# arneschneuing/DiffSBDD

Measured on NVIDIA H100. Metric: ligand_atoms_per_sec_500step_ddpm, higher is better.
Workload: dtype f32

## Files before the change

### diffsbdd_b200/csrc/dsb_tc.cu

```cuda
#include "dsb_tc.cuh"

namespace dsb {
using namespace tc;

__global__ void pack_b_image_kernel(float* __restrict__ hi, float* __restrict__ lo, const float* __restrict__ src, int lds,
                                    int scol, int n_rows, int n_dst_off, int K, int chunks, int TN) {
  const int64_t idx = (int64_t)blockIdx.x * blockDim.x + threadIdx.x;
  if (idx >= (int64_t)n_rows * K) return;
  const int n = (int)(idx / K), k = (int)(idx - (int64_t)n * K);
  const int nd = n_dst_off + n, nt = nd / TN, nl = nd % TN;
  const int kc = k / TKC, c = (k % TKC) >> 2, j = k & 3;
  const size_t off = ((size_t)nt * chunks + kc) * (size_t)(TN * TKC) + sw128_offset(nl, c) / 4 + j;
  const float w = src[(size_t)n * lds + scol + k];
  const float h = tf32_hi(w);
  hi[off] = h;
  lo[off] = w - h;
}

void launch_pack_b_image(float* hi, float* lo, const float* src, int lds, int scol, int n_rows, int n_dst_off, int K, int tn) {
  const int64_t tot = (int64_t)n_rows * K;
  pack_b_image_kernel<<<(unsigned)((tot + 255) / 256), 256>>>(hi, lo, src, lds, scol, n_rows, n_dst_off, K, K / TKC, tn);
}

__global__ void pack_b_image_f16_kernel(__half* __restrict__ hi, __half* __restrict__ lo, const float* __restrict__ src, int lds,
                                        int scol, int n_rows, int n_dst_off, int K, int chunks, float scale, int TN) {
  const int64_t idx = (int64_t)blockIdx.x * blockDim.x + threadIdx.x;
  if (idx >= (int64_t)n_rows * K) return;
  const int n = (int)(idx / K), k = (int)(idx - (int64_t)n * K);
  const int nd = n_dst_off + n, nt = nd / TN, nl = nd % TN;
  const int kc = k / TKC16, c16 = (k % TKC16) >> 3, j = k & 7;
  const size_t off = ((size_t)nt * chunks + kc) * (size_t)(TN * 64) + sw128_offset(nl, c16) / 2 + j;
  const float w = src[(size_t)n * lds + scol + k] * scale;
  const __half h = __float2half_rn(w);
  hi[off] = h;
  lo[off] = __float2half_rn(w - __half2float(h));
}

void launch_pack_b_image_f16(float* hi, float* lo, const float* src, int lds, int scol, int n_rows, int n_dst_off, int K, float scale, int tn) {
  const int64_t tot = (int64_t)n_rows * K;
  pack_b_image_f16_kernel<<<(unsigned)((tot + 255) / 256), 256>>>(reinterpret_cast<__half*>(hi), reinterpret_cast<__half*>(lo), src,
                                                                  lds, scol, n_rows, n_dst_off, K, K / TKC16, scale, tn);
}

__global__ void absmax_kernel(const float* __restrict__ src, int lds, int scol, int n_rows, int K, unsigned* __restrict__ out) {
  const int64_t idx = (int64_t)blockIdx.x * blockDim.x + threadIdx.x;
  float v = 0.f;
  if (idx < (int64_t)n_rows * K) { const int n = (int)(idx / K), k = (int)(idx - (int64_t)n * K); v = fabsf(src[(size_t)n * lds + scol + k]); }
#pragma unroll
  for (int o = 16; o > 0; o >>= 1) v = fmaxf(v, __shfl_xor_sync(0xffffffffu, v, o));
  if ((threadIdx.x & 31) == 0) atomicMax(out, __float_as_uint(v));
}
void launch_absmax(const float* src, int lds, int scol, int n_rows, int K, unsigned* out) {
  const int64_t tot = (int64_t)n_rows * K;
  absmax_kernel<<<(unsigned)((tot + 255) / 256), 256>>>(src, lds, scol, n_rows, K, out);
}

constexpr size_t kControlBytes = 128;
static_assert(sizeof(Control) <= kControlBytes, "Control block grew");
__device__ __forceinline__ char* align1024(uint8_t* raw) {
  return reinterpret_cast<char*>(raw) + ((1024u - (smem_u32(raw) & 1023u)) & 1023u);
}
template <int H> constexpr size_t tc_smem_base() { return 1024 + (size_t)NSTAGE * Geo<H>::STAGE_BYTES + kControlBytes; }

struct TcGemmArgs {
  const float* A1; int lda1; int K1;
  const float* A2; int lda2; int K2; float div2; const int32_t* deg2;
  const float* Bhi; const float* Blo;
  const float* bias; const float* R; int ldr;
  float* C; int ldc; int M; int Nn; int act;
  float* Z; int ldz;
  int dead_mt; int dead_nt;
  float inv_scale;
};

struct TileMap {
  int ntn, ntm, dead_mt, dead_nt, nA, n_live;
  __device__ TileMap(int M, int Nn, int dmt, int dnt, int TN) {
    ntn = Nn / TN; ntm = (M + TM - 1) / TM;
    dead_nt = dnt; dead_mt = dnt > 0 ? (dmt < ntm ? dmt : ntm) : ntm;
    nA = dead_mt * ntn;
    n_live = nA + (ntm - dead_mt) * (ntn - dead_nt);
  }
  __device__ void get(int t, int& mt, int& nt) const {
    if (t < nA) { mt = t / ntn; nt = t - mt * ntn; }
    else { const int u = t - nA, w = ntn - dead_nt; mt = dead_mt + u / w; nt = dead_nt + (u - (u / w) * w); }
  }
};

template <bool F16, int H>
__global__ void __launch_bounds__(TC_THREADS, 1) tc_node_gemm_kernel(TcGemmArgs g) {
  using G = Geo<H>;
  constexpr int TN = H, HPC = F16 ? 2 : 1;
  extern __shared__ uint8_t smem_raw[];
  char* const stages = align1024(smem_raw);
  Control* ctl = reinterpret_cast<Control*>(stages + NSTAGE * G::STAGE_BYTES);
  const int wg = threadIdx.x >> 7, warp = (threadIdx.x >> 5) & 3, lane = threadIdx.x & 31;
  const TileMap tm(g.M, g.Nn, g.dead_mt, g.dead_nt, TN);
  const int n_tiles = tm.n_live;
  const int n_my = ((int)blockIdx.x < n_tiles) ? (n_tiles - (int)blockIdx.x + (int)gridDim.x - 1) / (int)gridDim.x : 0;
  if (n_my == 0) return;
  const int K = g.K1 + g.K2, chunks = K / (F16 ? TKC16 : TKC);
  const uint32_t total = (uint32_t)(n_my * chunks);
  pdl_trigger();
  if (threadIdx.x == 0) control_init(ctl);
  __syncthreads();
  pdl_wait();
  const WeightStream<H> wst{ctl, stages};
  auto issue_w = [&](uint32_t q) {
    const int it = (int)(q / chunks), kc = (int)(q - (uint32_t)it * chunks);
    int mt, nt;
    tm.get(blockIdx.x + it * gridDim.x, mt, nt);
    const size_t off = ((size_t)nt * chunks + kc) * G::B_CHUNK_FLOATS;
    wst.issue(q, g.Bhi + off, g.Blo + off);
  };
  if (threadIdx.x >= MMA_THREADS) {
    regs_dec<WEIGHT_WG_REGS>();
    if (threadIdx.x == MMA_THREADS)
      for (uint32_t q = 0; q < total; ++q) issue_w(q);
    return;
  }
  regs_inc<MMA_WG_REGS>();

  const int sr = lane >> 3, pc = lane & 7;
  const int r0 = wg * WG_ROWS + 16 * warp + 4 * sr;
  const int re = wg * WG_ROWS + 16 * warp + (lane >> 2);
  const bool divides = g.div2 != 1.0f || g.deg2 != nullptr;
  float acc[G::ACC];
  MmaTracker trk;
  uint32_t q = 0;
  for (int it = 0; it < n_my; ++it) {
    int mt, nt;
    tm.get(blockIdx.x + it * gridDim.x, mt, nt);
    const int m0 = mt * TM, n0 = nt * TN;
    for (int kc = 0; kc < chunks; ++kc, ++q) {
      const int s = q & 1;
      char* st = stages + (size_t)s * G::STAGE_BYTES;
#pragma unroll
      for (int h = 0; h < HPC; ++h) {
        const int hf = kc * HPC + h, k = hf * TKC + 4 * pc;
        const bool second = k >= g.K1;
        float4 v[4];
#pragma unroll
        for (int i = 0; i < 4; ++i) {
          const int m = m0 + r0 + i;
          v[i] = make_float4(0.f, 0.f, 0.f, 0.f);
          if (m < g.M) v[i] = second ? *reinterpret_cast<const float4*>(g.A2 + (size_t)m * g.lda2 + (k - g.K1))
                                     : *reinterpret_cast<const float4*>(g.A1 + (size_t)m * g.lda1 + k);
        }
#pragma unroll
        for (int i = 0; i < 4; ++i) {
          float4 x = v[i];
          if (second && divides) {
            const int m = m0 + r0 + i;
            const float dv = g.deg2 ? (float)max(m < g.M ? g.deg2[m] : 1, 1) : g.div2;
            x.x = __fdiv_rn(x.x, dv); x.y = __fdiv_rn(x.y, dv); x.z = __fdiv_rn(x.z, dv); x.w = __fdiv_rn(x.w, dv);
          }
          store_pair<F16>(st + piece_offset<F16>(r0 + i, hf, pc), pk2(x.x, x.y), pk2(x.z, x.w));
        }
      }
      fence_proxy_async();
      wg_sync(wg);
      mbar_wait(&ctl->full_w[s], (q >> 1) & 1);
      wgmma_fence();
      mma_chunk<F16, H>(acc, st, wg, kc == 0);
      wgmma_commit();
      trk.after_commit<H>(ctl, acc, (int)q, kc == chunks - 1, lane == 0);
    }
    const f32x2 ip = pk2(g.inv_scale, g.inv_scale);
#pragma unroll
    for (int j = 0; j < H / 8; ++j) {
      const int n = n0 + 8 * j + 2 * (lane & 3);
      const f32x2 b = g.bias ? *reinterpret_cast<const float2*>(g.bias + n) : pk2(0.f, 0.f);
#pragma unroll
      for (int hh = 0; hh < 2; ++hh) {
        f32x2 x = pk2(acc[4 * j + 2 * hh], acc[4 * j + 2 * hh + 1]);
        x = F16 ? fma2(x, ip, b) : add2(x, b);
        if (g.act == 1) x = silu2(x);
        upk2(x, acc[4 * j + 2 * hh], acc[4 * j + 2 * hh + 1]);
      }
    }
    acc_fence(acc);
#pragma unroll
    for (int j = 0; j < H / 8; ++j) {
      const int n = n0 + 8 * j + 2 * (lane & 3);
#pragma unroll
      for (int hh = 0; hh < 2; ++hh) {
        const int row = m0 + re + 8 * hh;
        if (row < g.M) {
          f32x2 x = pk2(acc[4 * j + 2 * hh], acc[4 * j + 2 * hh + 1]);
          if (g.R) x = add2(*reinterpret_cast<const float2*>(g.R + (size_t)row * g.ldr + n), x);
          *reinterpret_cast<float2*>(g.C + (size_t)row * g.ldc + n) = x;
          if (g.Z) *reinterpret_cast<float2*>(g.Z + (size_t)row * g.ldz + n) = make_float2(0.f, 0.f);
        }
      }
    }
  }
}

template <int H>
struct EdgeExtra {
  float vec[2][3 * H];
  float wa[H];
  float d2[TM], d0[TM];
  int row[TM], col[TM], type[TM];
  float dir[3][TM];
};

struct TcEdgeArgs {
  const float* P; int ldp;
  const float4* x; const float4* cent; const int32_t* gid;
  const int32_t* vrow_ptr; const int32_t* vmap; int n_rows;
  const int32_t *erow, *ecol; const float* ed0; int NL;
  int nm;
  const float* W2hi[2]; const float* W2lo[2];
  const float* wr[2]; const float* wr0[2]; const float* tb[2]; const float* b2[2];
  const float* wa; const float* ba;
  float norm_constant, coords_range; int use_tanh;
  float* agg;
  float4* xagg;
  float inv_scale[2];
  float* part;
  int vcap;
};

template <bool COORD, int H>
__device__ __forceinline__ void edge_scalars(const TcEdgeArgs& a, EdgeExtra<H>* ex, int pr, int v0, int V, int m) {
  const int vr = v0 + pr;
  const int e = vr < V ? a.vmap[vr] : -1;
  int r = -1, c = 0, ty = 0; float d2 = 0.f, d0 = 0.f;
  float dir[3] = {0.f, 0.f, 0.f};
  if (e >= 0) {
    r = a.erow[e]; c = a.ecol[e]; d0 = a.ed0[e];
    const float4 xi = a.x[r], xj = a.x[c];
    const float dx = xi.x - xj.x, dy = xi.y - xj.y, dz = xi.z - xj.z;
    d2 = dx * dx + dy * dy + dz * dz;
    ty = (r < a.NL) == (c < a.NL) ? (r < a.NL ? 1 : 2) : 0;
    if (COORD) {
      if (m == 0) {
        const float den = sqrtf(d2 + 1e-8f) + a.norm_constant;
        dir[0] = dx / den; dir[1] = dy / den; dir[2] = dz / den;
      } else {
        const float4 mu = a.cent[a.gid[r]];
        const float ax = xi.x - mu.x, ay = xi.y - mu.y, az = xi.z - mu.z;
        const float bx = xj.x - mu.x, by = xj.y - mu.y, bz = xj.z - mu.z;
        const float cx = ay * bz - az * by, cy = az * bx - ax * bz, cz = ax * by - ay * bx;
        const float cn = sqrtf(cx * cx + cy * cy + cz * cz) + a.norm_constant;
        dir[0] = cx / cn; dir[1] = cy / cn; dir[2] = cz / cn;
      }
    }
  }
  ex->row[pr] = r; ex->col[pr] = c; ex->d2[pr] = d2; ex->d0[pr] = d0; ex->type[pr] = ty;
  if (COORD) {
#pragma unroll
    for (int k = 0; k < 3; ++k) ex->dir[k][pr] = dir[k];
  }
}

template <bool COORD, bool F16, int H, bool TB, bool DET = false>
__global__ void __launch_bounds__(TC_THREADS, 1) tc_edge_kernel(TcEdgeArgs a) {
  using G = Geo<H>;
  constexpr int HPC = F16 ? 2 : 1;
  constexpr int chunks = H / (TKC * HPC);
  extern __shared__ uint8_t smem_raw[];
  char* const stages = align1024(smem_raw);
  Control* ctl = reinterpret_cast<Control*>(stages + NSTAGE * G::STAGE_BYTES);
  EdgeExtra<H>* ex = reinterpret_cast<EdgeExtra<H>*>(reinterpret_cast<char*>(ctl) + kControlBytes);
  const int wg = threadIdx.x >> 7, wt = threadIdx.x & 127, warp = (threadIdx.x >> 5) & 3, lane = threadIdx.x & 31;
  const int nm = a.nm;

  pdl_trigger();
  for (int i = threadIdx.x; i < H; i += TC_THREADS) {
    for (int m = 0; m < nm; ++m) {
      float* v = ex->vec[m];
      v[i] = a.wr[m][i]; v[H + i] = a.wr0[m][i]; v[2 * H + i] = a.b2[m][i];
    }
    ex->wa[i] = a.wa ? a.wa[i] : 0.f;
  }
  if (threadIdx.x == 0) control_init(ctl);
  __syncthreads();
  pdl_wait();
  const int E = DET ? min(a.vrow_ptr[a.n_rows], a.vcap) : a.vrow_ptr[a.n_rows];
  const int n_units = ((E + TM - 1) / TM) * nm;
  const int n_my = ((int)blockIdx.x < n_units) ? (n_units - (int)blockIdx.x + (int)gridDim.x - 1) / (int)gridDim.x : 0;
  if (n_my == 0) return;
  auto unit_tile = [&](int j, int& m) { const int v = blockIdx.x + j * gridDim.x, t = v / nm; m = v - t * nm; return t; };
  const uint32_t total = (uint32_t)(n_my * chunks);
  const WeightStream<H> wst{ctl, stages};
  auto issue_w = [&](uint32_t q) {
    const int j = (int)(q / chunks), kc = (int)(q - (uint32_t)j * chunks);
    int m;
    unit_tile(j, m);
    wst.issue(q, a.W2hi[m] + (size_t)kc * G::B_CHUNK_FLOATS, a.W2lo[m] + (size_t)kc * G::B_CHUNK_FLOATS);
  };
  if (threadIdx.x >= MMA_THREADS) {
    regs_dec<WEIGHT_WG_REGS>();
    if (threadIdx.x == MMA_THREADS)
      for (uint32_t q = 0; q < total; ++q) issue_w(q);
    return;
  }
  regs_inc<MMA_WG_REGS>();

  const bool has_att = (!COORD) && a.wa != nullptr;
  const float ba = has_att ? a.ba[0] : 0.f;
  const int sr = lane >> 3, pc = lane & 7;
  const int r0 = wg * WG_ROWS + 16 * warp + 4 * sr;
  const int re = wg * WG_ROWS + 16 * warp + (lane >> 2);
  const float* const Pt = a.P + 4 * pc;
  const int soff = nm * H;
  float acc[G::ACC];
  MmaTracker trk;
  uint32_t q = 0;
  for (int j = 0; j < n_my; ++j) {
    int m;
    const int e0 = unit_tile(j, m) * TM;
    wg_sync(wg);
    if (wt < WG_ROWS) edge_scalars<COORD, H>(a, ex, wg * WG_ROWS + wt, e0, E, m);
    wg_sync(wg);
    const int moff = m * H;
    const float* pr = Pt + (size_t)max(ex->row[r0], 0) * a.ldp + moff;
    const float* ps[4];
    float pd2[4], pd0[4];
    int pty[4];
#pragma unroll
    for (int i = 0; i < 4; ++i) {
      ps[i] = Pt + (size_t)ex->col[r0 + i] * a.ldp + (soff + moff);
      pd2[i] = ex->d2[r0 + i]; pd0[i] = ex->d0[r0 + i];
      pty[i] = TB ? ex->type[r0 + i] * H : 0;
    }
    const float* wr = ex->vec[m] + 4 * pc;
    const float* wr0 = wr + H;
    const float* tbm = TB ? a.tb[m] + 4 * pc : nullptr;
#pragma unroll 1
    for (int kc = 0; kc < chunks; ++kc, ++q) {
      const int s = q & 1;
      char* st = stages + (size_t)s * G::STAGE_BYTES;
#pragma unroll
      for (int h = 0; h < HPC; ++h) {
        const int hf = kc * HPC + h;
        const float4 ga = *reinterpret_cast<const float4*>(pr + hf * TKC);
        float4 gb[4];
#pragma unroll
        for (int i = 0; i < 4; ++i) gb[i] = *reinterpret_cast<const float4*>(ps[i] + hf * TKC);
        const float4 r4 = *reinterpret_cast<const float4*>(wr + hf * TKC);
        const float4 r04 = *reinterpret_cast<const float4*>(wr0 + hf * TKC);
        const f32x2 a01 = pk2(ga.x, ga.y), a23 = pk2(ga.z, ga.w);
#pragma unroll
        for (int i = 0; i < 4; ++i) {
          const f32x2 d2p = pk2(pd2[i], pd2[i]), d0p = pk2(pd0[i], pd0[i]);
          f32x2 u01 = fma2(d0p, pk2(r04.x, r04.y), fma2(d2p, pk2(r4.x, r4.y), add2(a01, pk2(gb[i].x, gb[i].y))));
          f32x2 u23 = fma2(d0p, pk2(r04.z, r04.w), fma2(d2p, pk2(r4.z, r4.w), add2(a23, pk2(gb[i].z, gb[i].w))));
          if (TB) {
            const float4 t4 = *reinterpret_cast<const float4*>(tbm + pty[i] + hf * TKC);
            u01 = add2(u01, pk2(t4.x, t4.y)); u23 = add2(u23, pk2(t4.z, t4.w));
          }
          silu_pair<(DSB_SILU_PAIR & 1) != 0, (DSB_SILU_QUAD & 1) != 0>(u01, u23);
          store_pair<F16>(st + piece_offset<F16>(r0 + i, hf, pc), u01, u23);
        }
      }
      fence_proxy_async();
      wg_sync(wg);
      mbar_wait(&ctl->full_w[s], (q >> 1) & 1);
      wgmma_fence();
      mma_chunk<F16, H>(acc, st, wg, kc == 0);
      wgmma_commit();
      trk.after_commit<H>(ctl, acc, (int)q, kc == chunks - 1, lane == 0);
    }

    const float* b2 = ex->vec[m] + 2 * H;
    const f32x2 ip = pk2(a.inv_scale[m], a.inv_scale[m]);
    float s_lo = 0.f, s_hi = 0.f;
#pragma unroll
    for (int jj = 0; jj < H / 8; ++jj) {
      const int c = 8 * jj + 2 * (lane & 3);
      const f32x2 bb = *reinterpret_cast<const float2*>(b2 + c);
      const float2 ww = *reinterpret_cast<const float2*>(ex->wa + c);
      f32x2 lo = pk2(acc[4 * jj], acc[4 * jj + 1]), hi = pk2(acc[4 * jj + 2], acc[4 * jj + 3]);
      lo = F16 ? fma2(lo, ip, bb) : add2(lo, bb);
      hi = F16 ? fma2(hi, ip, bb) : add2(hi, bb);
      silu_pair<(DSB_SILU_PAIR & 2) != 0, (DSB_SILU_QUAD & 2) != 0>(lo, hi);
      upk2(lo, acc[4 * jj], acc[4 * jj + 1]); upk2(hi, acc[4 * jj + 2], acc[4 * jj + 3]);
      s_lo = fmaf(lo.y, ww.y, fmaf(lo.x, ww.x, s_lo));
      s_hi = fmaf(hi.y, ww.y, fmaf(hi.x, ww.x, s_hi));
    }
    s_lo += __shfl_xor_sync(0xffffffffu, s_lo, 1); s_lo += __shfl_xor_sync(0xffffffffu, s_lo, 2);
    s_hi += __shfl_xor_sync(0xffffffffu, s_hi, 1); s_hi += __shfl_xor_sync(0xffffffffu, s_hi, 2);
    const int row_lo = ex->row[re], row_hi = ex->row[re + 8];
    const int crow_lo = ex->row[re & ~3], crow_hi = ex->row[(re + 8) & ~3];
    const bool chunk_lane = (lane & 12) == 0;
    if constexpr (!COORD) {
      float g_lo = has_att ? sigmoid_f(s_lo + ba) : 1.0f, g_hi = has_att ? sigmoid_f(s_hi + ba) : 1.0f;
      g_lo = row_lo >= 0 ? g_lo : 0.f;
      g_hi = row_hi >= 0 ? g_hi : 0.f;
      float* const dst_lo = DET ? a.part + (size_t)((e0 + (re & ~3)) / kRowChunk) * H + 2 * (lane & 3)
                                : a.agg + (size_t)max(crow_lo, 0) * H + 2 * (lane & 3);
      float* const dst_hi = DET ? a.part + (size_t)((e0 + ((re + 8) & ~3)) / kRowChunk) * H + 2 * (lane & 3)
                                : a.agg + (size_t)max(crow_hi, 0) * H + 2 * (lane & 3);
#pragma unroll
      for (int jj = 0; jj < H / 8; ++jj) {
        float v0 = g_lo * acc[4 * jj], v1 = g_lo * acc[4 * jj + 1], v2 = g_hi * acc[4 * jj + 2], v3 = g_hi * acc[4 * jj + 3];
        v0 += __shfl_xor_sync(0xffffffffu, v0, 4); v1 += __shfl_xor_sync(0xffffffffu, v1, 4);
        v2 += __shfl_xor_sync(0xffffffffu, v2, 4); v3 += __shfl_xor_sync(0xffffffffu, v3, 4);
        v0 += __shfl_xor_sync(0xffffffffu, v0, 8); v1 += __shfl_xor_sync(0xffffffffu, v1, 8);
        v2 += __shfl_xor_sync(0xffffffffu, v2, 8); v3 += __shfl_xor_sync(0xffffffffu, v3, 8);
        if constexpr (DET)
          asm volatile("{\n\t.reg .pred p;\n\tsetp.ne.b32 p, %5, 0;\n\t"
                       "@p st.global.v2.f32 [%0], {%1, %2};\n\t"
                       "@p st.global.v2.f32 [%3], {%4, %6};\n\t}"
                       ::"l"(dst_lo + 8 * jj), "f"(v0), "f"(v1), "l"(dst_hi + 8 * jj), "f"(v2), "r"((int)chunk_lane), "f"(v3) : "memory");
        else
          asm volatile("{\n\t.reg .pred p;\n\tsetp.ne.b32 p, %5, 0;\n\t"
                       "@p red.global.add.v2.f32 [%0], {%1, %2};\n\t"
                       "@p red.global.add.v2.f32 [%3], {%4, %6};\n\t}"
                       ::"l"(dst_lo + 8 * jj), "f"(v0), "f"(v1), "l"(dst_hi + 8 * jj), "f"(v2), "r"((int)chunk_lane), "f"(v3) : "memory");
      }
    } else {
#pragma unroll
      for (int hh = 0; hh < 2; ++hh) {
        const int r = re + 8 * hh;
        const float sv = hh ? s_hi : s_lo;
        const bool live = (hh ? row_hi : row_lo) >= 0;
        float tr[3];
#pragma unroll
        for (int k = 0; k < 3; ++k) {
          const float d = ex->dir[k][r];
          float t;
          if (m == 0) t = a.use_tanh ? (d * tanhf(sv)) * a.coords_range : d * sv;
          else t = d * (a.use_tanh ? tanhf(sv) * a.coords_range : sv);
          t = live ? t : 0.f;
          t += __shfl_xor_sync(0xffffffffu, t, 4);
          t += __shfl_xor_sync(0xffffffffu, t, 8);
          tr[k] = t;
        }
        const int crow = hh ? crow_hi : crow_lo;
        if constexpr (DET) {
          if (chunk_lane && (lane & 3) == 0)
            reinterpret_cast<float4*>(a.part)[(size_t)((e0 + (r & ~3)) / kRowChunk) * nm + m] = make_float4(tr[0], tr[1], tr[2], 0.f);
        } else if (chunk_lane && (lane & 3) == 0 && crow >= 0) {
#pragma unroll
          for (int k = 0; k < 3; ++k) atomicAdd(reinterpret_cast<float*>(a.xagg) + (size_t)crow * 4 + k, tr[k]);
        }
      }
    }
  }
}

template <int H> static size_t gemm_smem_bytes() { return tc_smem_base<H>(); }
template <int H> static size_t edge_smem_bytes() {
  static_assert(tc_smem_base<H>() + sizeof(EdgeExtra<H>) <= 232448, "edge kernel exceeds the 227 KB of shared memory per CTA");
  return tc_smem_base<H>() + sizeof(EdgeExtra<H>);
}

bool tc_width_supported(int H) { return H == 128 || H == 192 || H == 256; }

template <typename Fn>
static int dispatch_width(int H, Fn&& fn) {
  switch (H) {
    case 128: return fn.template operator()<128>();
    case 192: return fn.template operator()<192>();
    case 256: return fn.template operator()<256>();
    default: set_error("tensor-core kernels exist for hidden_nf 128, 192, 256 (got %d)", H); return DSB_ERR_UNSUPPORTED_CONFIG;
  }
}

int configure_tc_kernels(int H) {
  return dispatch_width(H, [&]<int W>() -> int {
    const int gs = (int)gemm_smem_bytes<W>(), es = (int)edge_smem_bytes<W>();
    DSB_CUDA_OK(cudaFuncSetAttribute(tc_node_gemm_kernel<false, W>, cudaFuncAttributeMaxDynamicSharedMemorySize, gs));
    DSB_CUDA_OK(cudaFuncSetAttribute(tc_node_gemm_kernel<true, W>, cudaFuncAttributeMaxDynamicSharedMemorySize, gs));
    DSB_CUDA_OK(cudaFuncSetAttribute(tc_edge_kernel<false, false, W, false>, cudaFuncAttributeMaxDynamicSharedMemorySize, es));
    DSB_CUDA_OK(cudaFuncSetAttribute(tc_edge_kernel<false, false, W, true>, cudaFuncAttributeMaxDynamicSharedMemorySize, es));
    DSB_CUDA_OK(cudaFuncSetAttribute(tc_edge_kernel<false, true, W, false>, cudaFuncAttributeMaxDynamicSharedMemorySize, es));
    DSB_CUDA_OK(cudaFuncSetAttribute(tc_edge_kernel<false, true, W, true>, cudaFuncAttributeMaxDynamicSharedMemorySize, es));
    DSB_CUDA_OK(cudaFuncSetAttribute(tc_edge_kernel<true, false, W, false>, cudaFuncAttributeMaxDynamicSharedMemorySize, es));
    DSB_CUDA_OK(cudaFuncSetAttribute(tc_edge_kernel<true, false, W, true>, cudaFuncAttributeMaxDynamicSharedMemorySize, es));
    DSB_CUDA_OK(cudaFuncSetAttribute(tc_edge_kernel<true, true, W, false>, cudaFuncAttributeMaxDynamicSharedMemorySize, es));
    DSB_CUDA_OK(cudaFuncSetAttribute(tc_edge_kernel<true, true, W, true>, cudaFuncAttributeMaxDynamicSharedMemorySize, es));
    DSB_CUDA_OK(cudaFuncSetAttribute(tc_edge_kernel<false, false, W, false, true>, cudaFuncAttributeMaxDynamicSharedMemorySize, es));
    DSB_CUDA_OK(cudaFuncSetAttribute(tc_edge_kernel<false, false, W, true, true>, cudaFuncAttributeMaxDynamicSharedMemorySize, es));
    DSB_CUDA_OK(cudaFuncSetAttribute(tc_edge_kernel<false, true, W, false, true>, cudaFuncAttributeMaxDynamicSharedMemorySize, es));
    DSB_CUDA_OK(cudaFuncSetAttribute(tc_edge_kernel<false, true, W, true, true>, cudaFuncAttributeMaxDynamicSharedMemorySize, es));
    DSB_CUDA_OK(cudaFuncSetAttribute(tc_edge_kernel<true, false, W, false, true>, cudaFuncAttributeMaxDynamicSharedMemorySize, es));
    DSB_CUDA_OK(cudaFuncSetAttribute(tc_edge_kernel<true, false, W, true, true>, cudaFuncAttributeMaxDynamicSharedMemorySize, es));
    DSB_CUDA_OK(cudaFuncSetAttribute(tc_edge_kernel<true, true, W, false, true>, cudaFuncAttributeMaxDynamicSharedMemorySize, es));
    DSB_CUDA_OK(cudaFuncSetAttribute(tc_edge_kernel<true, true, W, true, true>, cudaFuncAttributeMaxDynamicSharedMemorySize, es));
    return 0;
  });
}

int launch_tc_node_gemm(const dsb_dynamics* d, const GemmArgs& g, const TcImage& w, int n_tile_off, bool f16, int32_t* status,
                        cudaStream_t s) {
  (void)status;
  if (g.M == 0) return 0;
  const int K = g.K1 + g.K2, TN = d->cfg.hidden_nf;
  if ((g.Nn % TN) || (K % TKC16) || (g.K1 % TKC16) || (g.lda1 % 4) || (g.ldc % 4)) {
    set_error("tc_node_gemm: unsupported shape K1=%d K2=%d Nn=%d", g.K1, g.K2, g.Nn);
    return DSB_ERR_INVALID_ARGUMENT;
  }
  TcGemmArgs a;
  a.A1 = g.A1; a.lda1 = g.lda1; a.K1 = g.K1; a.A2 = g.A2; a.lda2 = g.lda2; a.K2 = g.K2; a.div2 = g.div2; a.deg2 = g.deg2;
  const size_t img_off = (size_t)n_tile_off * (K / (f16 ? TKC16 : TKC)) * (size_t)(TN * TKC);
  a.Bhi = (f16 ? w.h_hi : w.t_hi) + img_off; a.Blo = (f16 ? w.h_lo : w.t_lo) + img_off;
  a.Z = g.Z; a.ldz = g.ldz;
  a.dead_nt = g.dead_cols / TN; a.dead_mt = a.dead_nt > 0 ? (g.dead_rows_from + TM - 1) / TM : 0;
  a.bias = g.bias; a.R = g.R; a.ldr = g.ldr; a.C = g.C; a.ldc = g.ldc; a.M = g.M; a.Nn = g.Nn; a.act = g.act;
  a.inv_scale = f16 ? w.h_inv : 1.0f;
  const int ntn_ = g.Nn / TN, ntm_ = (g.M + TM - 1) / TM;
  const int dmt_ = a.dead_nt > 0 ? (a.dead_mt < ntm_ ? a.dead_mt : ntm_) : ntm_;
  const int n_tiles = dmt_ * ntn_ + (ntm_ - dmt_) * (ntn_ - a.dead_nt);
  const int grid = n_tiles < d->num_sms ? n_tiles : d->num_sms;
  return dispatch_width(TN, [&]<int W>() -> int {
    DSB_CUDA_OK(launch_k(f16 ? tc_node_gemm_kernel<true, W> : tc_node_gemm_kernel<false, W>, grid, TC_THREADS, gemm_smem_bytes<W>(), s, a));
    return 0;
  });
}

int launch_tc_edge_gcl(const dsb_dynamics* d, const Dims& dm, const Workspace& ws, const GclW& w, const float4* x, PView pv, bool f16,
                       int32_t* status, cudaStream_t s) {
  (void)status;
  TcEdgeArgs a = {};
  a.P = pv.P; a.ldp = pv.ldp; a.x = x; a.cent = ws.cent; a.gid = ws.gid; a.vrow_ptr = ws.vrow_ptr; a.vmap = ws.vmap; a.n_rows = dm.N;
  a.erow = ws.erow; a.ecol = ws.ecol; a.ed0 = ws.ed0; a.NL = dm.NL; a.nm = 1;
  a.W2hi[0] = f16 ? w.iW2.h_hi : w.iW2.t_hi; a.W2lo[0] = f16 ? w.iW2.h_lo : w.iW2.t_lo;
  a.inv_scale[0] = f16 ? w.iW2.h_inv : 1.0f; a.inv_scale[1] = 1.0f;
  a.wr[0] = w.wr; a.wr0[0] = w.wr0; a.tb[0] = w.tb; a.b2[0] = w.b2;
  a.wa = w.wa; a.ba = w.ba; a.agg = ws.agg; a.part = ws.part; a.vcap = ws.vcap;
  const bool det = d->deterministic != 0;
  return dispatch_width(d->cfg.hidden_nf, [&]<int W>() -> int {
    auto kern = w.tb ? (f16 ? tc_edge_kernel<false, true, W, true> : tc_edge_kernel<false, false, W, true>)
                     : (f16 ? tc_edge_kernel<false, true, W, false> : tc_edge_kernel<false, false, W, false>);
    if (det)
      kern = w.tb ? (f16 ? tc_edge_kernel<false, true, W, true, true> : tc_edge_kernel<false, false, W, true, true>)
                  : (f16 ? tc_edge_kernel<false, true, W, false, true> : tc_edge_kernel<false, false, W, false, true>);
    DSB_CUDA_OK(launch_k(kern, d->num_sms, TC_THREADS, edge_smem_bytes<W>(), s, a));
    return 0;
  });
}

int launch_tc_edge_coord(const dsb_dynamics* d, const Dims& dm, const Workspace& ws, const EquivW& w, const float4* x, PView pv, bool f16,
                         int32_t* status, cudaStream_t s) {
  (void)status;
  const dsb_config& c = d->cfg;
  TcEdgeArgs a = {};
  a.nm = c.reflection_equivariant ? 1 : 2;
  a.P = pv.P; a.ldp = pv.ldp; a.x = x; a.cent = ws.cent; a.gid = ws.gid; a.vrow_ptr = ws.vrow_ptr; a.vmap = ws.vmap; a.n_rows = dm.n_coord_rows;
  a.erow = ws.erow; a.ecol = ws.ecol; a.ed0 = ws.ed0; a.NL = dm.NL;
  a.inv_scale[0] = a.inv_scale[1] = 1.0f;
  for (int m = 0; m < a.nm; ++m) {
    a.W2hi[m] = f16 ? w.iW2[m].h_hi : w.iW2[m].t_hi; a.W2lo[m] = f16 ? w.iW2[m].h_lo : w.iW2[m].t_lo;
    a.inv_scale[m] = f16 ? w.iW2[m].h_inv : 1.0f;
    a.wr[m] = w.wr[m]; a.wr0[m] = w.wr0[m]; a.tb[m] = w.tb[m]; a.b2[m] = w.b2[m];
  }
  a.wa = w.w3; a.ba = nullptr;
  a.norm_constant = c.norm_constant; a.coords_range = c.coords_range; a.use_tanh = c.tanh; a.xagg = ws.xagg; a.part = ws.part; a.vcap = ws.vcap;
  const bool det = d->deterministic != 0;
  return dispatch_width(c.hidden_nf, [&]<int W>() -> int {
    auto kern = w.tb[0] ? (f16 ? tc_edge_kernel<true, true, W, true> : tc_edge_kernel<true, false, W, true>)
                        : (f16 ? tc_edge_kernel<true, true, W, false> : tc_edge_kernel<true, false, W, false>);
    if (det)
      kern = w.tb[0] ? (f16 ? tc_edge_kernel<true, true, W, true, true> : tc_edge_kernel<true, false, W, true, true>)
                     : (f16 ? tc_edge_kernel<true, true, W, false, true> : tc_edge_kernel<true, false, W, false, true>);
    DSB_CUDA_OK(launch_k(kern, d->num_sms, TC_THREADS, edge_smem_bytes<W>(), s, a));
    return 0;
  });
}

}
```

### diffsbdd_b200/csrc/dsb_tc.cuh

```cuda
#pragma once
#include <cuda_fp16.h>

#include "dsb_internal.cuh"
#include "dsb_wgmma.cuh"

namespace dsb {
namespace tc {

constexpr int TM = 128;
constexpr int WG_ROWS = 64;
constexpr int TKC = 32;
constexpr int TKC16 = 64;
constexpr float X_SCALE = 1.0f;
constexpr int A_CHUNK_BYTES = TM * 128;
constexpr int NSTAGE = 2;
constexpr int MMA_THREADS = 256;
constexpr int TC_THREADS = MMA_THREADS + 128;
constexpr int WEIGHT_WG_REGS = 40, MMA_WG_REGS = 232;
template <int R> __device__ __forceinline__ void regs_dec() { asm volatile("setmaxnreg.dec.sync.aligned.u32 %0;" ::"n"(R)); }
template <int R> __device__ __forceinline__ void regs_inc() { asm volatile("setmaxnreg.inc.sync.aligned.u32 %0;" ::"n"(R)); }

template <int H>
struct Geo {
  static_assert(H == 128 || H == 192 || H == 256, "tensor-core kernels are built for hidden_nf 128, 192, 256");
  static constexpr int TN = H;
  static constexpr int ACC = H / 2;
  static constexpr int B_CHUNK_BYTES = H * 128;
  static constexpr int B_CHUNK_FLOATS = H * TKC;
  static constexpr int STAGE_BYTES = 2 * A_CHUNK_BYTES + 2 * B_CHUNK_BYTES;
};

__device__ __forceinline__ uint32_t smem_u32(const void* p) { return (uint32_t)__cvta_generic_to_shared(p); }

__device__ __forceinline__ void mbar_init(uint64_t* bar, uint32_t count) {
  asm volatile("mbarrier.init.shared::cta.b64 [%0], %1;" ::"r"(smem_u32(bar)), "r"(count) : "memory");
}
__device__ __forceinline__ void mbar_arrive(uint64_t* bar) {
  asm volatile("mbarrier.arrive.shared::cta.b64 _, [%0];" ::"r"(smem_u32(bar)) : "memory");
}
__device__ __forceinline__ void mbar_arrive_expect_tx(uint64_t* bar, uint32_t bytes) {
  asm volatile("mbarrier.arrive.expect_tx.shared::cta.b64 _, [%0], %1;" ::"r"(smem_u32(bar)), "r"(bytes) : "memory");
}
__device__ __forceinline__ bool mbar_try_wait(uint64_t* bar, uint32_t parity) {
  uint32_t ok;
  asm volatile(
      "{\n\t.reg .pred P1;\n\t"
      "mbarrier.try_wait.parity.shared::cta.b64 P1, [%1], %2, %3;\n\t"
      "selp.b32 %0, 1, 0, P1;\n\t}"
      : "=r"(ok)
      : "r"(smem_u32(bar)), "r"(parity), "r"(20000u)
      : "memory");
  return ok != 0;
}
__device__ __forceinline__ void mbar_wait(uint64_t* bar, uint32_t parity) {
  uint32_t spins = 0;
  while (!mbar_try_wait(bar, parity)) {
    ++spins;
    asm volatile("{\n\t.reg .pred p;\n\tsetp.gt.u32 p, %0, %1;\n\t@p trap;\n\t}" ::"r"(spins), "r"(1u << 17));
  }
}
__device__ __forceinline__ void fence_barrier_init() { asm volatile("fence.mbarrier_init.release.cluster;" ::: "memory"); }
__device__ __forceinline__ void fence_proxy_async() { asm volatile("fence.proxy.async.shared::cta;" ::: "memory"); }
__device__ __forceinline__ void wg_sync(int wg) { asm volatile("bar.sync %0, 128;" ::"r"(wg + 1) : "memory"); }

__device__ __forceinline__ void bulk_g2s(void* smem_dst, const void* gmem_src, uint32_t bytes, uint64_t* bar) {
  asm volatile("cp.async.bulk.shared::cluster.global.mbarrier::complete_tx::bytes [%0], [%1], %2, [%3];"
               ::"r"(smem_u32(smem_dst)), "l"(gmem_src), "r"(bytes), "r"(smem_u32(bar)) : "memory");
}

__device__ __forceinline__ uint64_t wgmma_desc_sw128(uint32_t smem_addr) {
  return (uint64_t)((smem_addr >> 4) & 0x3FFFu) | (1ull << 16) | ((uint64_t)(1024 >> 4) << 32) | (1ull << 62);
}
__device__ __forceinline__ void wgmma_fence() { asm volatile("wgmma.fence.sync.aligned;" ::: "memory"); }
__device__ __forceinline__ void wgmma_commit() { asm volatile("wgmma.commit_group.sync.aligned;" ::: "memory"); }
template <int N>
__device__ __forceinline__ void wgmma_wait() { asm volatile("wgmma.wait_group.sync.aligned %0;" ::"n"(N) : "memory"); }
template <int R>
__device__ __forceinline__ void acc_fence(float (&d)[R]) {
#pragma unroll
  for (int i = 0; i < R; ++i) asm volatile("" : "+f"(d[i])::"memory");
}

template <bool F16, int H>
__device__ __forceinline__ void mma_chunk(float (&d)[H / 2], const char* st, int wg, bool first_chunk) {
  using G = Geo<H>;
  const uint32_t xhi = smem_u32(st) + (uint32_t)(wg * WG_ROWS * 128), xlo = xhi + A_CHUNK_BYTES;
  const uint32_t whi = smem_u32(st) + 2 * A_CHUNK_BYTES, wlo = whi + G::B_CHUNK_BYTES;
#pragma unroll
  for (int ks = 0; ks < 4; ++ks) {
    const uint32_t ko = ks * 32;
    const uint32_t acc = (first_chunk && ks == 0) ? 0u : 1u;
    if constexpr (F16) {
      Wgmma<H>::f16(d, wgmma_desc_sw128(xlo + ko), wgmma_desc_sw128(whi + ko), acc);
      Wgmma<H>::f16(d, wgmma_desc_sw128(xhi + ko), wgmma_desc_sw128(wlo + ko), 1u);
      Wgmma<H>::f16(d, wgmma_desc_sw128(xhi + ko), wgmma_desc_sw128(whi + ko), 1u);
    } else {
      Wgmma<H>::tf32(d, wgmma_desc_sw128(xlo + ko), wgmma_desc_sw128(whi + ko), acc);
      Wgmma<H>::tf32(d, wgmma_desc_sw128(xhi + ko), wgmma_desc_sw128(wlo + ko), 1u);
      Wgmma<H>::tf32(d, wgmma_desc_sw128(xhi + ko), wgmma_desc_sw128(whi + ko), 1u);
    }
  }
}

__device__ __forceinline__ float tf32_hi(float x) { return __uint_as_float((__float_as_uint(x) + 0x1000u) & 0xffffe000u); }

__device__ __host__ __forceinline__ uint32_t sw128_offset(int r, int c) {
  return (uint32_t)((r >> 3) * 1024 + (r & 7) * 128 + ((c ^ (r & 7)) << 4));
}

__device__ __forceinline__ void residual_f16(uint32_t hi2, float x0, float x1, float& r0, float& r1) {
  const __half2 h = *reinterpret_cast<const __half2*>(&hi2);
  r0 = x0 - __low2float(h);
  r1 = x1 - __high2float(h);
}
__device__ __forceinline__ uint32_t h2_bits(__half2 h) { return *reinterpret_cast<const uint32_t*>(&h); }

template <bool F16>
__device__ __forceinline__ void store_pair(char* dst, f32x2 u01, f32x2 u23) {
  float x0, x1, x2, x3;
  upk2(u01, x0, x1); upk2(u23, x2, x3);
  if constexpr (F16) {
    const __half2 h0 = __floats2half2_rn(x0, x1), h1 = __floats2half2_rn(x2, x3);
    float l0, l1, l2, l3;
    residual_f16(h2_bits(h0), x0, x1, l0, l1); residual_f16(h2_bits(h1), x2, x3, l2, l3);
    const __half2 q0 = __floats2half2_rn(l0, l1), q1 = __floats2half2_rn(l2, l3);
    uint2 hv, lv;
    hv.x = h2_bits(h0); hv.y = h2_bits(h1);
    lv.x = h2_bits(q0); lv.y = h2_bits(q1);
    *reinterpret_cast<uint2*>(dst) = hv;
    *reinterpret_cast<uint2*>(dst + A_CHUNK_BYTES) = lv;
  } else {
    const float4 h = make_float4(tf32_hi(x0), tf32_hi(x1), tf32_hi(x2), tf32_hi(x3));
    *reinterpret_cast<float4*>(dst) = h;
    *reinterpret_cast<float4*>(dst + A_CHUNK_BYTES) = make_float4(x0 - h.x, x1 - h.y, x2 - h.z, x3 - h.w);
  }
}
template <bool F16>
__device__ __forceinline__ uint32_t piece_offset(int r, int hf, int p) {
  return F16 ? sw128_offset(r, (hf & 1) * 4 + (p >> 1)) + (uint32_t)(p & 1) * 8u : sw128_offset(r, p);
}

struct Control {
  uint64_t full_w[NSTAGE];
  uint64_t empty[NSTAGE];
};

__device__ __forceinline__ void control_init(Control* c) {
  for (int s = 0; s < NSTAGE; ++s) { mbar_init(&c->full_w[s], 1); mbar_init(&c->empty[s], 8); }
  fence_barrier_init();
}

template <int H>
struct WeightStream {
  Control* ctl;
  char* stages;
  __device__ void issue(uint32_t g, const float* hi, const float* lo) const {
    using G = Geo<H>;
    const int s = g & 1;
    if (g >= NSTAGE) mbar_wait(&ctl->empty[s], ((g >> 1) - 1) & 1);
    char* st = stages + (size_t)s * G::STAGE_BYTES + 2 * A_CHUNK_BYTES;
    mbar_arrive_expect_tx(&ctl->full_w[s], 2 * G::B_CHUNK_BYTES);
    bulk_g2s(st, hi, G::B_CHUNK_BYTES, &ctl->full_w[s]);
    bulk_g2s(st + G::B_CHUNK_BYTES, lo, G::B_CHUNK_BYTES, &ctl->full_w[s]);
  }
};

struct MmaTracker {
  int pend = -1;
  template <int H>
  __device__ __forceinline__ void after_commit(Control* ctl, float (&d)[H / 2], int g, bool last_of_tile, bool leader) {
    if (last_of_tile) {
      wgmma_wait<0>();
      acc_fence(d);
      if (leader) { if (pend >= 0) mbar_arrive(&ctl->empty[pend & 1]); mbar_arrive(&ctl->empty[g & 1]); }
      pend = -1;
    } else {
      wgmma_wait<1>();
      if (leader && pend >= 0) mbar_arrive(&ctl->empty[pend & 1]);
      pend = g;
    }
  }
};

}
}
```

Before: 704.7.

## Software-pipeline edge scalar loads and A-tile build across MMA chunks

Restructures the edge kernel loop so that building the next chunk's A tile and the next unit's edge scalars (split into four latency-hiding steps, stored in double-buffered smem) overlap with the in-flight wgmma. The wait-for-all is moved to a drain after the last chunk, and the first chunk of the next unit is built before draining. Also rewrites the scatter reduction as a transpose-style shuffle so every lane issues one red/store per pair of columns, with no predicated half-idle stores. This adds register pressure, smem for two scalar buffers, and more complex synchronization. It also requires chunks >= 2.

```diff
diff --git a/diffsbdd_b200/csrc/dsb_tc.cu b/diffsbdd_b200/csrc/dsb_tc.cu
--- a/diffsbdd_b200/csrc/dsb_tc.cu
+++ b/diffsbdd_b200/csrc/dsb_tc.cu
@@ -164,8 +164,9 @@
       wgmma_fence();
       mma_chunk<F16, H>(acc, st, wg, kc == 0);
       wgmma_commit();
-      trk.after_commit<H>(ctl, acc, (int)q, kc == chunks - 1, lane == 0);
-    }
+      trk.release_prev(ctl, (int)q, lane == 0);
+    }
+    trk.drain<H>(ctl, acc, lane == 0);
     const f32x2 ip = pk2(g.inv_scale, g.inv_scale);
 #pragma unroll
     for (int j = 0; j < H / 8; ++j) {
@@ -197,13 +198,17 @@
   }
 }
 
+struct EdgeScalars {
+  float d2[TM], d0[TM];
+  int row[TM], col[TM], type[TM];
+  float dir[3][TM];
+};
+
 template <int H>
 struct EdgeExtra {
   float vec[2][3 * H];
   float wa[H];
-  float d2[TM], d0[TM];
-  int row[TM], col[TM], type[TM];
-  float dir[3][TM];
+  EdgeScalars sc[2];
 };
 
 struct TcEdgeArgs {
@@ -223,38 +228,49 @@
   int vcap;
 };
 
-template <bool COORD, int H>
-__device__ __forceinline__ void edge_scalars(const TcEdgeArgs& a, EdgeExtra<H>* ex, int pr, int v0, int V, int m) {
-  const int vr = v0 + pr;
-  const int e = vr < V ? a.vmap[vr] : -1;
-  int r = -1, c = 0, ty = 0; float d2 = 0.f, d0 = 0.f;
-  float dir[3] = {0.f, 0.f, 0.f};
-  if (e >= 0) {
-    r = a.erow[e]; c = a.ecol[e]; d0 = a.ed0[e];
-    const float4 xi = a.x[r], xj = a.x[c];
-    const float dx = xi.x - xj.x, dy = xi.y - xj.y, dz = xi.z - xj.z;
-    d2 = dx * dx + dy * dy + dz * dz;
-    ty = (r < a.NL) == (c < a.NL) ? (r < a.NL ? 1 : 2) : 0;
-    if (COORD) {
-      if (m == 0) {
-        const float den = sqrtf(d2 + 1e-8f) + a.norm_constant;
-        dir[0] = dx / den; dir[1] = dy / den; dir[2] = dz / den;
-      } else {
-        const float4 mu = a.cent[a.gid[r]];
-        const float ax = xi.x - mu.x, ay = xi.y - mu.y, az = xi.z - mu.z;
-        const float bx = xj.x - mu.x, by = xj.y - mu.y, bz = xj.z - mu.z;
-        const float cx = ay * bz - az * by, cy = az * bx - ax * bz, cz = ax * by - ay * bx;
-        const float cn = sqrtf(cx * cx + cy * cy + cz * cz) + a.norm_constant;
-        dir[0] = cx / cn; dir[1] = cy / cn; dir[2] = cz / cn;
+template <bool COORD>
+struct ScalarSteps {
+  int e, r, c, gi;
+  float d0;
+  float4 xi, xj;
+  __device__ __forceinline__ void step(int k, const TcEdgeArgs& a, EdgeScalars* sc, int pr, int v0, int V, int m) {
+    if (k == 0) {
+      const int vr = v0 + pr;
+      e = a.vmap[min(vr, V - 1)];
+      e = vr < V ? e : -1;
+    } else if (k == 1) {
+      const int ec = max(e, 0);
+      r = a.erow[ec]; c = a.ecol[ec]; d0 = a.ed0[ec];
+      r = e >= 0 ? r : 0; c = e >= 0 ? c : 0;
+    } else if (k == 2) {
+      xi = a.x[r]; xj = a.x[c];
+      if (COORD) gi = a.gid[r];
+    } else {
+      const bool live = e >= 0;
+      const float dx = xi.x - xj.x, dy = xi.y - xj.y, dz = xi.z - xj.z;
+      const float d2 = dx * dx + dy * dy + dz * dz;
+      const int ty = (r < a.NL) == (c < a.NL) ? (r < a.NL ? 1 : 2) : 0;
+      sc->row[pr] = live ? r : -1; sc->col[pr] = c; sc->d2[pr] = live ? d2 : 0.f; sc->d0[pr] = live ? d0 : 0.f;
+      sc->type[pr] = live ? ty : 0;
+      if (COORD) {
+        float dir[3];
+        if (m == 0) {
+          const float den = sqrtf(d2 + 1e-8f) + a.norm_constant;
+          dir[0] = dx / den; dir[1] = dy / den; dir[2] = dz / den;
+        } else {
+          const float4 mu = a.cent[gi];
+          const float ax = xi.x - mu.x, ay = xi.y - mu.y, az = xi.z - mu.z;
+          const float bx = xj.x - mu.x, by = xj.y - mu.y, bz = xj.z - mu.z;
+          const float cx = ay * bz - az * by, cy = az * bx - ax * bz, cz = ax * by - ay * bx;
+          const float cn = sqrtf(cx * cx + cy * cy + cz * cz) + a.norm_constant;
+          dir[0] = cx / cn; dir[1] = cy / cn; dir[2] = cz / cn;
+        }
+#pragma unroll
+        for (int k = 0; k < 3; ++k) sc->dir[k][pr] = live ? dir[k] : 0.f;
       }
     }
   }
-  ex->row[pr] = r; ex->col[pr] = c; ex->d2[pr] = d2; ex->d0[pr] = d0; ex->type[pr] = ty;
-  if (COORD) {
-#pragma unroll
-    for (int k = 0; k < 3; ++k) ex->dir[k][pr] = dir[k];
-  }
-}
+};
 
 template <bool COORD, bool F16, int H, bool TB, bool DET = false>
 __global__ void __launch_bounds__(TC_THREADS, 1) tc_edge_kernel(TcEdgeArgs a) {
@@ -307,64 +323,82 @@
   const int re = wg * WG_ROWS + 16 * warp + (lane >> 2);
   const float* const Pt = a.P + 4 * pc;
   const int soff = nm * H;
+  auto build = [&](const EdgeScalars* sc, int m, int kc, int s) {
+    char* st = stages + (size_t)s * G::STAGE_BYTES;
+    const int moff = m * H;
+    const float* pr = Pt + (size_t)max(sc->row[r0], 0) * a.ldp + moff;
+    const int4 cl = *reinterpret_cast<const int4*>(sc->col + r0);
+    const float4 d2v = *reinterpret_cast<const float4*>(sc->d2 + r0), d0v = *reinterpret_cast<const float4*>(sc->d0 + r0);
+    const int4 tyv = *reinterpret_cast<const int4*>(sc->type + r0);
+    const float* const ps[4] = {Pt + (size_t)cl.x * a.ldp + (soff + moff), Pt + (size_t)cl.y * a.ldp + (soff + moff),
+                                Pt + (size_t)cl.z * a.ldp + (soff + moff), Pt + (size_t)cl.w * a.ldp + (soff + moff)};
+    const float pd2[4] = {d2v.x, d2v.y, d2v.z, d2v.w}, pd0[4] = {d0v.x, d0v.y, d0v.z, d0v.w};
+    const int pty[4] = {TB ? tyv.x * H : 0, TB ? tyv.y * H : 0, TB ? tyv.z * H : 0, TB ? tyv.w * H : 0};
+    const float* wr = ex->vec[m] + 4 * pc;
+    const float* wr0 = wr + H;
+    const float* tbm = TB ? a.tb[m] + 4 * pc : nullptr;
+#pragma unroll
+    for (int h = 0; h < HPC; ++h) {
+      const int hf = kc * HPC + h;
+      const float4 ga = *reinterpret_cast<const float4*>(pr + hf * TKC);
+      float4 gb[4];
+#pragma unroll
+      for (int i = 0; i < 4; ++i) gb[i] = *reinterpret_cast<const float4*>(ps[i] + hf * TKC);
+      const float4 r4 = *reinterpret_cast<const float4*>(wr + hf * TKC);
+      const float4 r04 = *reinterpret_cast<const float4*>(wr0 + hf * TKC);
+      const f32x2 a01 = pk2(ga.x, ga.y), a23 = pk2(ga.z, ga.w);
+#pragma unroll
+      for (int i = 0; i < 4; ++i) {
+        const f32x2 d2p = pk2(pd2[i], pd2[i]), d0p = pk2(pd0[i], pd0[i]);
+        f32x2 u01 = fma2(d0p, pk2(r04.x, r04.y), fma2(d2p, pk2(r4.x, r4.y), add2(a01, pk2(gb[i].x, gb[i].y))));
+        f32x2 u23 = fma2(d0p, pk2(r04.z, r04.w), fma2(d2p, pk2(r4.z, r4.w), add2(a23, pk2(gb[i].z, gb[i].w))));
+        if (TB) {
+          const float4 t4 = *reinterpret_cast<const float4*>(tbm + pty[i] + hf * TKC);
+          u01 = add2(u01, pk2(t4.x, t4.y)); u23 = add2(u23, pk2(t4.z, t4.w));
+        }
+        silu_pair<(DSB_SILU_PAIR & 1) != 0, (DSB_SILU_QUAD & 1) != 0>(u01, u23);
+        store_pair<F16>(st + piece_offset<F16>(r0 + i, hf, pc), u01, u23);
+      }
+    }
+  };
   float acc[G::ACC];
   MmaTracker trk;
   uint32_t q = 0;
+  auto issue = [&](int kc) {
+    const int s = q & 1;
+    fence_proxy_async();
+    wg_sync(wg);
+    mbar_wait(&ctl->full_w[s], (q >> 1) & 1);
+    wgmma_fence();
+    mma_chunk<F16, H>(acc, stages + (size_t)s * G::STAGE_BYTES, wg, kc == 0);
+    wgmma_commit();
+    trk.release_prev(ctl, (int)q, lane == 0);
+    ++q;
+  };
+  static_assert(chunks >= 2, "the scalar steps of the next unit need at least one chunk before the last");
+  constexpr int kSteps = 4;
+  const int psc = wg * WG_ROWS + (wt & (WG_ROWS - 1));
+  ScalarSteps<COORD> stp;
+  int m;
+  int e0 = unit_tile(0, m) * TM;
+  for (int k = 0; k < kSteps; ++k) stp.step(k, a, &ex->sc[0], psc, e0, E, m);
+  wg_sync(wg);
+  build(&ex->sc[0], m, 0, 0);
   for (int j = 0; j < n_my; ++j) {
-    int m;
-    const int e0 = unit_tile(j, m) * TM;
-    wg_sync(wg);
-    if (wt < WG_ROWS) edge_scalars<COORD, H>(a, ex, wg * WG_ROWS + wt, e0, E, m);
-    wg_sync(wg);
-    const int moff = m * H;
-    const float* pr = Pt + (size_t)max(ex->row[r0], 0) * a.ldp + moff;
-    const float* ps[4];
-    float pd2[4], pd0[4];
-    int pty[4];
-#pragma unroll
-    for (int i = 0; i < 4; ++i) {
-      ps[i] = Pt + (size_t)ex->col[r0 + i] * a.ldp + (soff + moff);
-      pd2[i] = ex->d2[r0 + i]; pd0[i] = ex->d0[r0 + i];
-      pty[i] = TB ? ex->type[r0 + i] * H : 0;
-    }
-    const float* wr = ex->vec[m] + 4 * pc;
-    const float* wr0 = wr + H;
-    const float* tbm = TB ? a.tb[m] + 4 * pc : nullptr;
-#pragma unroll 1
-    for (int kc = 0; kc < chunks; ++kc, ++q) {
-      const int s = q & 1;
-      char* st = stages + (size_t)s * G::STAGE_BYTES;
-#pragma unroll
-      for (int h = 0; h < HPC; ++h) {
-        const int hf = kc * HPC + h;
-        const float4 ga = *reinterpret_cast<const float4*>(pr + hf * TKC);
-        float4 gb[4];
-#pragma unroll
-        for (int i = 0; i < 4; ++i) gb[i] = *reinterpret_cast<const float4*>(ps[i] + hf * TKC);
-        const float4 r4 = *reinterpret_cast<const float4*>(wr + hf * TKC);
-        const float4 r04 = *reinterpret_cast<const float4*>(wr0 + hf * TKC);
-        const f32x2 a01 = pk2(ga.x, ga.y), a23 = pk2(ga.z, ga.w);
-#pragma unroll
-        for (int i = 0; i < 4; ++i) {
-          const f32x2 d2p = pk2(pd2[i], pd2[i]), d0p = pk2(pd0[i], pd0[i]);
-          f32x2 u01 = fma2(d0p, pk2(r04.x, r04.y), fma2(d2p, pk2(r4.x, r4.y), add2(a01, pk2(gb[i].x, gb[i].y))));
-          f32x2 u23 = fma2(d0p, pk2(r04.z, r04.w), fma2(d2p, pk2(r4.z, r4.w), add2(a23, pk2(gb[i].z, gb[i].w))));
-          if (TB) {
-            const float4 t4 = *reinterpret_cast<const float4*>(tbm + pty[i] + hf * TKC);
-            u01 = add2(u01, pk2(t4.x, t4.y)); u23 = add2(u23, pk2(t4.z, t4.w));
-          }
-          silu_pair<(DSB_SILU_PAIR & 1) != 0, (DSB_SILU_QUAD & 1) != 0>(u01, u23);
-          store_pair<F16>(st + piece_offset<F16>(r0 + i, hf, pc), u01, u23);
-        }
-      }
-      fence_proxy_async();
-      wg_sync(wg);
-      mbar_wait(&ctl->full_w[s], (q >> 1) & 1);
-      wgmma_fence();
-      mma_chunk<F16, H>(acc, st, wg, kc == 0);
-      wgmma_commit();
-      trk.after_commit<H>(ctl, acc, (int)q, kc == chunks - 1, lane == 0);
-    }
+    const EdgeScalars* sc = &ex->sc[j & 1];
+    EdgeScalars* sc_next = &ex->sc[(j + 1) & 1];
+    int m_next;
+    const int e0_next = unit_tile(j + 1, m_next) * TM;
+#pragma unroll (F16 ? chunks : 1)
+    for (int kc = 0; kc < chunks - 1; ++kc) {
+      issue(kc);
+      for (int k = kc * kSteps / (chunks - 1); k < (kc + 1) * kSteps / (chunks - 1); ++k)
+        stp.step(k, a, sc_next, psc, e0_next, E, m_next);
+      build(sc, m, kc + 1, q & 1);
+    }
+    issue(chunks - 1);
+    build(sc_next, m_next, 0, q & 1);
+    trk.drain<H>(ctl, acc, lane == 0);
 
     const float* b2 = ex->vec[m] + 2 * H;
     const f32x2 ip = pk2(a.inv_scale[m], a.inv_scale[m]);
@@ -384,34 +418,32 @@
     }
     s_lo += __shfl_xor_sync(0xffffffffu, s_lo, 1); s_lo += __shfl_xor_sync(0xffffffffu, s_lo, 2);
     s_hi += __shfl_xor_sync(0xffffffffu, s_hi, 1); s_hi += __shfl_xor_sync(0xffffffffu, s_hi, 2);
-    const int row_lo = ex->row[re], row_hi = ex->row[re + 8];
-    const int crow_lo = ex->row[re & ~3], crow_hi = ex->row[(re + 8) & ~3];
+    const int row_lo = sc->row[re], row_hi = sc->row[re + 8];
+    const int crow_lo = sc->row[re & ~3], crow_hi = sc->row[(re + 8) & ~3];
     const bool chunk_lane = (lane & 12) == 0;
     if constexpr (!COORD) {
       float g_lo = has_att ? sigmoid_f(s_lo + ba) : 1.0f, g_hi = has_att ? sigmoid_f(s_hi + ba) : 1.0f;
       g_lo = row_lo >= 0 ? g_lo : 0.f;
       g_hi = row_hi >= 0 ? g_hi : 0.f;
-      float* const dst_lo = DET ? a.part + (size_t)((e0 + (re & ~3)) / kRowChunk) * H + 2 * (lane & 3)
-                                : a.agg + (size_t)max(crow_lo, 0) * H + 2 * (lane & 3);
-      float* const dst_hi = DET ? a.part + (size_t)((e0 + ((re + 8) & ~3)) / kRowChunk) * H + 2 * (lane & 3)
-                                : a.agg + (size_t)max(crow_hi, 0) * H + 2 * (lane & 3);
-#pragma unroll
-      for (int jj = 0; jj < H / 8; ++jj) {
-        float v0 = g_lo * acc[4 * jj], v1 = g_lo * acc[4 * jj + 1], v2 = g_hi * acc[4 * jj + 2], v3 = g_hi * acc[4 * jj + 3];
-        v0 += __shfl_xor_sync(0xffffffffu, v0, 4); v1 += __shfl_xor_sync(0xffffffffu, v1, 4);
-        v2 += __shfl_xor_sync(0xffffffffu, v2, 4); v3 += __shfl_xor_sync(0xffffffffu, v3, 4);
-        v0 += __shfl_xor_sync(0xffffffffu, v0, 8); v1 += __shfl_xor_sync(0xffffffffu, v1, 8);
-        v2 += __shfl_xor_sync(0xffffffffu, v2, 8); v3 += __shfl_xor_sync(0xffffffffu, v3, 8);
+      const bool hi_half = (lane & 4) != 0, odd_group = (lane & 8) != 0;
+      const int crow = hi_half ? crow_hi : crow_lo;
+      const int chunk_row = hi_half ? (re + 8) & ~3 : re & ~3;
+      float* const dst = (DET ? a.part + (size_t)((e0 + chunk_row) / kRowChunk) * H : a.agg + (size_t)max(crow, 0) * H)
+                         + 2 * (lane & 3) + (odd_group ? 8 : 0);
+#pragma unroll
+      for (int jj = 0; jj < H / 8; jj += 2) {
+        const float lo[4] = {g_lo * acc[4 * jj], g_lo * acc[4 * jj + 1], g_lo * acc[4 * jj + 4], g_lo * acc[4 * jj + 5]};
+        const float hi[4] = {g_hi * acc[4 * jj + 2], g_hi * acc[4 * jj + 3], g_hi * acc[4 * jj + 6], g_hi * acc[4 * jj + 7]};
+        float t[4];
+#pragma unroll
+        for (int k = 0; k < 4; ++k) t[k] = (hi_half ? hi[k] : lo[k]) + __shfl_xor_sync(0xffffffffu, hi_half ? lo[k] : hi[k], 4);
+        float u[2];
+#pragma unroll
+        for (int k = 0; k < 2; ++k) u[k] = (odd_group ? t[2 + k] : t[k]) + __shfl_xor_sync(0xffffffffu, odd_group ? t[k] : t[2 + k], 8);
         if constexpr (DET)
-          asm volatile("{\n\t.reg .pred p;\n\tsetp.ne.b32 p, %5, 0;\n\t"
-                       "@p st.global.v2.f32 [%0], {%1, %2};\n\t"
-                       "@p st.global.v2.f32 [%3], {%4, %6};\n\t}"
-                       ::"l"(dst_lo + 8 * jj), "f"(v0), "f"(v1), "l"(dst_hi + 8 * jj), "f"(v2), "r"((int)chunk_lane), "f"(v3) : "memory");
+          asm volatile("st.global.v2.f32 [%0], {%1, %2};" ::"l"(dst + 8 * jj), "f"(u[0]), "f"(u[1]) : "memory");
         else
-          asm volatile("{\n\t.reg .pred p;\n\tsetp.ne.b32 p, %5, 0;\n\t"
-                       "@p red.global.add.v2.f32 [%0], {%1, %2};\n\t"
-                       "@p red.global.add.v2.f32 [%3], {%4, %6};\n\t}"
-                       ::"l"(dst_lo + 8 * jj), "f"(v0), "f"(v1), "l"(dst_hi + 8 * jj), "f"(v2), "r"((int)chunk_lane), "f"(v3) : "memory");
+          asm volatile("red.global.add.v2.f32 [%0], {%1, %2};" ::"l"(dst + 8 * jj), "f"(u[0]), "f"(u[1]) : "memory");
       }
     } else {
 #pragma unroll
@@ -422,7 +454,7 @@
         float tr[3];
 #pragma unroll
         for (int k = 0; k < 3; ++k) {
-          const float d = ex->dir[k][r];
+          const float d = sc->dir[k][r];
           float t;
           if (m == 0) t = a.use_tanh ? (d * tanhf(sv)) * a.coords_range : d * sv;
           else t = d * (a.use_tanh ? tanhf(sv) * a.coords_range : sv);
@@ -441,6 +473,7 @@
         }
       }
     }
+    m = m_next; e0 = e0_next;
   }
 }
 
diff --git a/diffsbdd_b200/csrc/dsb_tc.cuh b/diffsbdd_b200/csrc/dsb_tc.cuh
--- a/diffsbdd_b200/csrc/dsb_tc.cuh
+++ b/diffsbdd_b200/csrc/dsb_tc.cuh
@@ -167,18 +167,17 @@
 
 struct MmaTracker {
   int pend = -1;
+  __device__ __forceinline__ void release_prev(Control* ctl, int g, bool leader) {
+    wgmma_wait<1>();
+    if (leader && pend >= 0) mbar_arrive(&ctl->empty[pend & 1]);
+    pend = g;
+  }
   template <int H>
-  __device__ __forceinline__ void after_commit(Control* ctl, float (&d)[H / 2], int g, bool last_of_tile, bool leader) {
-    if (last_of_tile) {
-      wgmma_wait<0>();
-      acc_fence(d);
-      if (leader) { if (pend >= 0) mbar_arrive(&ctl->empty[pend & 1]); mbar_arrive(&ctl->empty[g & 1]); }
-      pend = -1;
-    } else {
-      wgmma_wait<1>();
-      if (leader && pend >= 0) mbar_arrive(&ctl->empty[pend & 1]);
-      pend = g;
-    }
+  __device__ __forceinline__ void drain(Control* ctl, float (&d)[H / 2], bool leader) {
+    wgmma_wait<0>();
+    acc_fence(d);
+    if (leader && pend >= 0) mbar_arrive(&ctl->empty[pend & 1]);
+    pend = -1;
   }
 };
 
```

Result: faster. 760.8, median of 6 (+8.0%).
